# mims-harvard/GNNDelete

Hardware: AMD Instinct MI355X
Metric: Del-op train iters/sec (higher is better)
Workload: dtype f32; 1 GPU; synth-collab GCN 2-layer, 5.0% IN edge deletion, full-graph Del step (both_layerwise, mse_mean); num_nodes=235868, in_dim=128, hidden_dim=128, out_dim=64, train_edges_undirected=2122296, df_edges=53057, sdf_edges=1602188, spmm_nnz=1838056, S1=178921, S2=188697, hip_graph=True, matrix_products=fp32 matrix instruction (v_mfma_f32_32x32x2_f32), parallelism=single, ranks_seen=1

## Files before the change

### gnndelete_amd/_lib.py

```python
import ctypes
import os
import re

_HERE = os.path.dirname(os.path.abspath(__file__))
LIB_PATH = os.environ.get('GNNDELETE_HIP_LIB') or os.path.join(_HERE, 'lib', 'libgnndelete_hip.so')
HEADER_PATH = os.path.join(os.path.dirname(_HERE), 'include', 'gnndelete_hip.h')

_i32, _i64, _f32, _f64, _p = ctypes.c_int32, ctypes.c_int64, ctypes.c_float, ctypes.c_double, ctypes.c_void_p

ABI_VERSION = 9

PROTOTYPES = {
    'gd_abi_version': (ctypes.c_int, []),
    'gd_last_error_string': (ctypes.c_char_p, []),
    'gd_build_source_hash': (ctypes.c_char_p, []),
    'gd_matrix_split': (ctypes.c_int, []),
    'gd_set_matrix_split': (ctypes.c_int, [ctypes.c_int]),
    'gd_csr_from_coo_workspace': (_i64, [_i32, _i64]),
    'gd_csr_from_coo': (ctypes.c_int, [_p, _p, _i64, _i32, _p, _p, _p, _p, _p, _i64, _p]),
    'gd_gcn_norm_f32': (ctypes.c_int, [_p, _p, _i32, _p, _p]),
    'gd_spmm_csr_f32': (ctypes.c_int, [_p, _p, _p, _p, _i64, _p, _i64, _p, _f32, _i32, _i32, _p]),
    'gd_spmm_csr_balanced_f32': (ctypes.c_int, [_p, _i32, _p, _i32, _p, _p, _p, _i64, _p, _i64, _p, _f32, _p, _p, _i32,
                                                _i32, _i32, _p, _p]),
    'gd_spmm_csr_onepass_f32': (ctypes.c_int, [_p, _i32, _p, _p, _p, _i64, _p, _i64, _p, _f32, _p, _i32, _i32, _i32, _p, _p]),
# ... 46 lines not shown
    'gd_batch_loss_terms_workspace': (_i64, [_i32, _i64]),
    'gd_batch_loss_terms': (ctypes.c_int, [_p, _i64, _p, _i64, _i32, _p, _i32, _i32, _f32, _f32, _p, _p, _p, _p, _p, _i64, _p]),
    'gd_rowpair_mse_workspace': (_i64, [_i32]),
    'gd_rowpair_mse_f32': (ctypes.c_int, [_p, _i64, _p, _i64, _i32, _p, _p, _i32, _p, _p, _p, _p, _i64, _i32,
                                          _p, _p, _p]),
    'gd_rowtarget_mse_workspace': (_i64, [_i32]),
    'gd_rowtarget_mse_f32': (ctypes.c_int, [_p, _i64, _p, _i32, _p, _p, _p, _p, _i32, _p, _i64, _p, _p, _p]),
    'gd_rowtarget_mse_pair_covers': (ctypes.c_int32, [_i32, _i32]),
    'gd_rowtarget_mse_pair_f32': (ctypes.c_int, [_p, _i64, _p, _i32, _p, _p, _p, _p, _i32, _p, _i64, _p, _p, _i64, _p, _i32, _p, _p, _p, _p, _i32, _p, _i64, _p, _p]),
    'gd_gemm_f32_workspace': (_i64, [_i32, _i32, _i32]),
    'gd_gemm_f32': (ctypes.c_int, [_p, _i64, _p, _i32, _p, _i32, _i32, _p, _p, _i64, _p, _p]),
    'gd_edge_dot_f32': (ctypes.c_int, [_p, _i64, _i32, _p, _p, _p, _i64, _p, _i64, _p, _p]),
    'gd_edge_dot_bwd_f32': (ctypes.c_int, [_p, _i64, _i32, _p, _p, _p, _i64, _p, _p, _i64, _p, _i64, _p]),
    'gd_rows_gemm_wgrad_adam_f32': (ctypes.c_int, [_p, _i64, _p, _p, _i64, _p, _p, _p, _i32, _i32, _i32, _p, _i32, _p,
                                                   _p, _p, _p, _p, _f64, _f64, _f64, _f64, _p]),
    'gd_rows_gemm_wgrad_blocks': (_i32, [_i32]),
    'gd_rows_gemm_wgrad_loss_f32': (ctypes.c_int, [_p, _i64, _p, _p, _i64, _p, _p, _p, _p, _p, _p, _i32, _i32, _i32, _p, _i32,
                                                   _p, _p, _p, _p, _p, _p, _f64, _f64, _f64, _f64, _p]),
    'gd_del_loss_bwd_blocks': (_i32, [_i32]),
    'gd_del_loss_bwd_f32': (ctypes.c_int, [_p, _i64, _p, _i32, _p, _i32, _p, _p, _p, _p, _p, _i64, _p, _i64, _p, _p]),
    'gd_del_loss_bwd_wgrad_f32': (ctypes.c_int, [_p, _i64, _p, _i32, _p, _i32, _p, _p, _p, _p, _p, _i64, _p, _i64, _p, _p, _p]),
    'gd_del_loss_bwd_wgrad_parts': (ctypes.c_int32, [_i32, _i32]),
    'gd_del_loss_bwd_wgrad_parts_f32': (ctypes.c_int, [_p, _i64, _p, _i32, _p, _i32, _p, _p, _p, _p, _p, _i64, _p, _i64, _p, _p, _i32, _p]),
    'gd_del1_loss_wgrad_covers': (ctypes.c_int32, [_i32, _i32]),
    'gd_del1_loss_wgrad_parts': (ctypes.c_int32, [_i32]),
    'gd_del1_chain_loss_wgrad_f32': (ctypes.c_int, [_p, _i64, _p, _i32, _p, _i32, _p, _i64, _p, _p, _p, _p, _p, _p, _i64, _i32, _p, _p, _p, _p, _p, _p, _p, _i32, _p]),
    'gd_del1_loss_wgrad_f32': (ctypes.c_int, [_p, _i64, _p, _i32, _p, _i32, _p, _i64, _p, _p, _p, _p, _p, _p, _i64, _p, _p, _i32, _p]),
    'gd_rowtarget_mse_blocks': (_i32, [_i32]),
    'gd_rowfold_loss_blocks': (_i32, [_i32]),
    'gd_rowfold_loss_f32': (ctypes.c_int, [_i32, _p, _i64, _p, _i32, _i32, _p, _p, _p, _p, _i32, _p, _i64, _p, _p]),
    'gd_rowfold_kld_scale_f32': (ctypes.c_int, [_p, _i32, _f32, _f32, _f32, _f32, _p, _p, _i32, _i32, _p, _i64, _p, _p]),
    'gd_loss_finalize_f32': (ctypes.c_int, [_p, _i32, _p, _i32, _p, _p, _i32, _p, _p, _p]),
    'gd_pairs_sigmoid_mse_workspace': (_i64, [_i32, _i32]),
    'gd_pairs_sigmoid_mse_f32': (ctypes.c_int, [_p, _i64, _p, _i32, _i32, _p, _i64, _f32, _p, _p, _p, _p]),
    'gd_edgeprob_dec_workspace': (_i64, [_i64, _i32]),
    'gd_edgeprob_dec_f32': (ctypes.c_int, [_p, _i64, _i64, _i32, _p, _i64, _p, _i64, _i64, _f32, _p, _p, _p, _p, _p, _p, _p]),
    'gd_edge_incidence_workspace': (_i64, [_i64, _i64]),
    'gd_edge_incidence': (ctypes.c_int, [_p, _p, _i64, _i64, _p, _p, _p, _p, _i64, _p]),
    'gd_rows_add_f32': (ctypes.c_int, [_p, _i64, _i64, _p, _i32, _p, _i64, _f32, _i32, _p]),
    'gd_edgeprob_record_f32': (ctypes.c_int, [_p, _p, _f32, _f32, _p, _i32, _p, _p]),
    'gd_edge_bce_workspace': (_i64, [_i64, _i32]),
    'gd_edge_bce_f32': (ctypes.c_int, [_p, _i64, _i64, _i32, _p, _i64, _i64, _p, _i64, _i64, _f32, _p, _p, _p, _p, _p, _p, _p]),
    'gd_col_sum_workspace': (_i64, [_i64, _i32]),
    'gd_col_sum_f32': (ctypes.c_int, [_p, _i64, _i64, _i32, _p, _p, _p, _p, _p, _p]),
    'gd_row_nll_workspace': (_i64, [_i64, _i32]),
    'gd_row_nll_f32': (ctypes.c_int, [_p, _i64, _i64, _i32, _i32, _p, _i64, _p, _f32, _p, _i64, _p, _p, _p]),
# ... 74 lines not shown
```

### gnndelete_amd/csrc/del_fused.hip

```cpp
#include <stdlib.h>

#include "common.h"

namespace gd {

using f32x16 = __attribute__((ext_vector_type(16))) float;

struct DelLoss {
  const int32_t* slot;
  const float* tm;
  const float* coef;
  const float* cnt_signed;
  float* partials;
};

template <int NT, bool WG>
__global__ __launch_bounds__(256, (NT == 2 && WG) ? 1 : 2) void del_loss_bwd_kernel(const float* __restrict__ p, int64_t ld_p,
                                                              const int32_t* __restrict__ idx, int32_t n_sel,
                                                              const float* __restrict__ w, DelLoss loss,
                                                              float* __restrict__ dz, int64_t ld_dz,
                                                              float* __restrict__ dp, int64_t ld_dp,
                                                              float* __restrict__ wg_partials) {
  constexpr int D = 32 * NT;
  constexpr int PB = D + 4;
// ... 199 lines not shown
    float* const red = wl;
#pragma unroll
    for (int mt = 0; mt < NT; ++mt)
#pragma unroll
      for (int nt = 0; nt < NT; ++nt)
#pragma unroll
        for (int r = 0; r < 16; ++r)
          red[wave * D * D + (32 * mt + (r & 3) + 8 * (r >> 2) + 4 * kh) * D + 32 * nt + lo] = gacc[mt * NT + nt][r];
    __syncthreads();
    float* const out = wg_partials + (int64_t)blockIdx.x * D * D;
    for (int e = tid; e < D * D; e += 256) out[e] = (red[e] + red[D * D + e]) + (red[2 * D * D + e] + red[3 * D * D + e]);
  }
  ls0 = wave_sum(ls0);
  ls1 = wave_sum(ls1);
  if (lane == 0) { lred[0][wave] = ls0; lred[1][wave] = ls1; }
  __syncthreads();
  if (tid == 0) {
    loss.partials[2 * blockIdx.x + 0] = (lred[0][0] + lred[0][1]) + (lred[0][2] + lred[0][3]);
    loss.partials[2 * blockIdx.x + 1] = (lred[1][0] + lred[1][1]) + (lred[1][2] + lred[1][3]);
  }
}

typedef float f32x4w __attribute__((ext_vector_type(4)));
template <bool HAS_DZ>
__global__ __launch_bounds__(256) __attribute__((amdgpu_waves_per_eu(1, 1))) void del_loss_bwd_ws_kernel(
    const float* __restrict__ p, int64_t ld_p, const int32_t* __restrict__ idx, int32_t n_sel, const float* __restrict__ w,
    DelLoss loss, float* __restrict__ dz, int64_t ld_dz, float* __restrict__ dp, int64_t ld_dp, float* __restrict__ wg_partials,
    int32_t n_part) {
  constexpr int D = 64, PT = 80;
  extern __shared__ __attribute__((aligned(16))) float wl[];
  __shared__ float lred[2][4];
  const int tid = threadIdx.x, lane = tid & 63;
  const int wave = __builtin_amdgcn_readfirstlane(tid >> 6);
  const int r = lane & 15, kq = lane >> 4;
  float* const tp = wl + wave * (2 * 16 * PT);
  float* const tz = tp + 16 * PT;
  const int n_units = (n_sel + 15) >> 4;
  const int n_waves = gridDim.x * 4, wid = blockIdx.x * 4 + wave;
  const int u_lo = (int)((int64_t)n_units * wid / n_waves), u_hi = (int)((int64_t)n_units * (wid + 1) / n_waves);

  auto slot_of = [&](int u) -> int { return min(min(u, n_units - 1) * 16 + r, n_sel - 1); };
  int32_t row_n = idx[slot_of(u_lo)], ls_n = loss.slot[slot_of(u_lo)];
  int32_t row_nn = idx[slot_of(u_lo + 1)], ls_nn = loss.slot[slot_of(u_lo + 1)];
  __builtin_amdgcn_sched_barrier(0);
  float wr1[4][16], wr2[4][16];
#pragma unroll
  for (int t = 0; t < 4; ++t)
#pragma unroll
    for (int s_ = 0; s_ < 16; ++s_) wr1[t][s_] = w[(kq * 16 + s_) * D + 16 * t + r];
#pragma unroll
  for (int t2 = 0; t2 < 4; ++t2)
#pragma unroll
    for (int t = 0; t < 4; ++t) {
      const float4 f = *reinterpret_cast<const float4*>(w + (16 * t2 + r) * D + 16 * t + 4 * kq);
      wr2[t2][4 * t + 0] = f.x; wr2[t2][4 * t + 1] = f.y; wr2[t2][4 * t + 2] = f.z; wr2[t2][4 * t + 3] = f.w;
    }
  f32x4w gacc[16];
#pragma unroll
  for (int i = 0; i < 16; ++i) gacc[i] = f32x4w{0.f, 0.f, 0.f, 0.f};
  float ls0 = 0.f, ls1 = 0.f;

  float4 x[4], tv[4];
  float cf_raw, cn_raw;
  int32_t ls_cur;
  auto fetch_targets = [&](int32_t u) {
    const int uc = max(u, 0);
    const float* trow = loss.tm + (int64_t)uc * D + 4 * kq;
#pragma unroll
    for (int t = 0; t < 4; ++t) tv[t] = *reinterpret_cast<const float4*>(trow + 16 * t);
    cf_raw = loss.coef[uc];
    cn_raw = loss.cnt_signed[uc];
    ls_cur = u;
  };
  auto fetch_rows = [&](int32_t row) {
    const float4* src = reinterpret_cast<const float4*>(p + (int64_t)row * ld_p + kq * 16);
#pragma unroll
    for (int i = 0; i < 4; ++i) x[i] = src[i];
  };
  float a_op[4][4], b_op[4][4];
// ... 14 lines not shown
    fetch_rows(row_n);
    fetch_targets(ls_n);
    for (int u = u_lo; u < u_hi; ++u) {
      const int32_t row = row_n;
      const int s_a = min(u, n_units - 1) * 16 + r;
      const float livef = s_a < n_sel ? 1.f : 0.f;
      row_n = row_nn;
      ls_n = ls_nn;
      row_nn = idx[slot_of(u + 2)];
      ls_nn = loss.slot[slot_of(u + 2)];
      f32x4w acc[4];
#pragma unroll
      for (int i = 0; i < 4; ++i) {
        const float xv[4] = {x[i].x, x[i].y, x[i].z, x[i].w};
#pragma unroll
        for (int c = 0; c < 4; ++c)
#pragma unroll
          for (int t = 0; t < 4; ++t) {
            if (i == 0 && c == 0) acc[t] = __builtin_amdgcn_mfma_f32_16x16x4f32(wr1[t][0], xv[0], f32x4w{0.f, 0.f, 0.f, 0.f}, 0, 0, 0);
            else acc[t] = __builtin_amdgcn_mfma_f32_16x16x4f32(wr1[t][4 * i + c], xv[c], acc[t], 0, 0, 0);
          }
      }
      __builtin_amdgcn_sched_barrier(0);
      p3();
      const float cf = ls_cur >= 0 ? cf_raw : 0.f, cn = ls_cur >= 0 ? cn_raw : 0.f;
      float sq = 0.f;
      f32x4w g[4];
#pragma unroll
      for (int t = 0; t < 4; ++t) {
        const float4 d4 = make_float4(acc[t][0] - tv[t].x, acc[t][1] - tv[t].y, acc[t][2] - tv[t].z, acc[t][3] - tv[t].w);
        sq = fmaf(d4.x, d4.x, sq); sq = fmaf(d4.y, d4.y, sq); sq = fmaf(d4.z, d4.z, sq); sq = fmaf(d4.w, d4.w, sq);
        g[t] = f32x4w{cf * d4.x, cf * d4.y, cf * d4.z, cf * d4.w};
        if (HAS_DZ) *reinterpret_cast<float4*>(dz + (int64_t)min(s_a, n_sel - 1) * ld_dz + 16 * t + 4 * kq) = make_float4(g[t][0], g[t][1], g[t][2], g[t][3]);
        *reinterpret_cast<float4*>(tz + r * PT + 16 * t + 4 * kq) = make_float4(livef * g[t][0], livef * g[t][1], livef * g[t][2], livef * g[t][3]);
      }
      sq *= livef;
      if (cn >= 0.f) ls0 = fmaf(cn, sq, ls0); else ls1 = fmaf(-cn, sq, ls1);
#pragma unroll
      for (int i = 0; i < 4; ++i) *reinterpret_cast<float4*>(tp + r * PT + kq * 16 + 4 * i) = x[i];
      __builtin_amdgcn_sched_barrier(0);
      fetch_targets(ls_n);
      fetch_rows(row_n);
      __builtin_amdgcn_fence(__ATOMIC_ACQ_REL, "wavefront");
      __builtin_amdgcn_wave_barrier();
#pragma unroll
      for (int sp = 0; sp < 4; ++sp)
#pragma unroll
        for (int t = 0; t < 4; ++t) {
          a_op[sp][t] = tp[(4 * sp + kq) * PT + 16 * t + r];
          b_op[sp][t] = tz[(4 * sp + kq) * PT + 16 * t + r];
        }
      __builtin_amdgcn_sched_barrier(0);
      f32x4w dacc[4];
#pragma unroll
      for (int t = 0; t < 4; ++t)
#pragma unroll
        for (int c = 0; c < 4; ++c)
#pragma unroll
          for (int t2 = 0; t2 < 4; ++t2) {
            if (t == 0 && c == 0) dacc[t2] = __builtin_amdgcn_mfma_f32_16x16x4f32(wr2[t2][0], g[0][0], f32x4w{0.f, 0.f, 0.f, 0.f}, 0, 0, 0);
            else dacc[t2] = __builtin_amdgcn_mfma_f32_16x16x4f32(wr2[t2][4 * t + c], g[t][c], dacc[t2], 0, 0, 0);
          }
      __builtin_amdgcn_sched_barrier(0);
      {
        float* orow = dp + (int64_t)row * ld_dp + 4 * kq;
#pragma unroll
        for (int t2 = 0; t2 < 4; ++t2) *reinterpret_cast<float4*>(orow + 16 * t2) = make_float4(dacc[t2][0], dacc[t2][1], dacc[t2][2], dacc[t2][3]);
      }
      __builtin_amdgcn_fence(__ATOMIC_ACQ_REL, "wavefront");
      __builtin_amdgcn_wave_barrier();
      __builtin_amdgcn_sched_barrier(0);
    }
    p3();
  }
  __syncthreads();
  float* const red = wl;
#pragma unroll
  for (int ta = 0; ta < 4; ++ta)
#pragma unroll
    for (int tb = 0; tb < 4; ++tb)
#pragma unroll
      for (int v = 0; v < 4; ++v) red[wave * D * D + (16 * ta + 4 * kq + v) * D + 16 * tb + r] = gacc[ta * 4 + tb][v];
  __syncthreads();
  for (int slot = blockIdx.x; slot < n_part; slot += gridDim.x) {
    float* const out = wg_partials + (int64_t)slot * D * D;
    const bool mine = slot == (int)blockIdx.x;
    for (int e = tid; e < D * D; e += 256) out[e] = mine ? (red[e] + red[D * D + e]) + (red[2 * D * D + e] + red[3 * D * D + e]) : 0.f;
  }
  ls0 = wave_sum(ls0);
  ls1 = wave_sum(ls1);
  if (lane == 0) { lred[0][wave] = ls0; lred[1][wave] = ls1; }
  __syncthreads();
  if (tid == 0) {
    for (int slot = blockIdx.x; slot < n_part; slot += gridDim.x) {
      const bool mine = slot == (int)blockIdx.x;
      loss.partials[2 * slot + 0] = mine ? (lred[0][0] + lred[0][1]) + (lred[0][2] + lred[0][3]) : 0.f;
// ... 423 lines not shown
  hipStream_t s = (hipStream_t)stream;
  const DelLoss loss{loss_slot, tm, coef, cnt_signed, loss_partials};
  if (!with_wgrad) {
    const dim3 grid(del_fused_grid(n_sel));
    const size_t lds = ((size_t)d * d + (size_t)d * (d + 4)) * sizeof(float);
    switch (d / 32) {
      case 1: hipLaunchKernelGGL((del_loss_bwd_kernel<1, false>), grid, dim3(256), lds, s, p, ld_p, idx, n_sel, w, loss, dz, ld_dz, dp, ld_dp, nullptr); break;
      default: hipLaunchKernelGGL((del_loss_bwd_kernel<2, false>), grid, dim3(256), lds, s, p, ld_p, idx, n_sel, w, loss, dz, ld_dz, dp, ld_dp, nullptr); break;
    }
    return launched("del_loss_bwd");
  }
  static const bool ws_on = [] { const char* e = getenv("GD_DEL2_WS"); return !(e && atoi(e) == 0); }();
  if (ws_on && d == 64 && n_sel >= 65536) {
    const int n_all = gd_rows_gemm_wgrad_blocks(n_sel);
    const int n_part = n_part_req > 0 ? n_part_req : n_all;
    GD_REQUIRE(n_part <= n_all && n_part >= (ws_cu_count() < n_all ? ws_cu_count() : n_all), GD_E_DIM,
               "%s: n_part=%d outside [gd_del_loss_bwd_wgrad_parts, gd_rows_gemm_wgrad_blocks = %d]", name, n_part, n_all);
    const int grid_ws = ws_cu_count() < n_part ? ws_cu_count() : n_part;
    constexpr int kLdsWs = 4 * 64 * 64 * 4;
    if (dz) {
      static const hipError_t a1 = hipFuncSetAttribute(reinterpret_cast<const void*>(&del_loss_bwd_ws_kernel<true>), hipFuncAttributeMaxDynamicSharedMemorySize, kLdsWs);
      if (a1 != hipSuccess) return fail(-(int)a1, "gd_del_loss_bwd_wgrad_f32: %s", hipGetErrorString(a1));
      hipLaunchKernelGGL((del_loss_bwd_ws_kernel<true>), dim3(grid_ws), dim3(256), kLdsWs, s, p, ld_p, idx, n_sel, w, loss, dz, ld_dz, dp, ld_dp,
                         wgrad_partials, n_part);
    } else {
      static const hipError_t a0 = hipFuncSetAttribute(reinterpret_cast<const void*>(&del_loss_bwd_ws_kernel<false>), hipFuncAttributeMaxDynamicSharedMemorySize, kLdsWs);
      if (a0 != hipSuccess) return fail(-(int)a0, "gd_del_loss_bwd_wgrad_f32: %s", hipGetErrorString(a0));
      hipLaunchKernelGGL((del_loss_bwd_ws_kernel<false>), dim3(grid_ws), dim3(256), kLdsWs, s, p, ld_p, idx, n_sel, w, loss, dz, ld_dz, dp, ld_dp,
                         wgrad_partials, n_part);
    }
    return launched("del_loss_bwd_ws");
  }
  GD_REQUIRE(n_part_req == 0 || n_part_req == gd_rows_gemm_wgrad_blocks(n_sel), GD_E_DIM,
             "%s: n_part=%d but this size leaves gd_rows_gemm_wgrad_blocks(n_sel) = %d partials", name, n_part_req, gd_rows_gemm_wgrad_blocks(n_sel));
  const dim3 grid(gd_rows_gemm_wgrad_blocks(n_sel));
#define GD_DF_CASE(NT_)                                                                                                        \
  do {                                                                                                                         \
    constexpr int kD = 32 * NT_;                                                                                               \
    constexpr int kLds = (kD * kD + kD * (kD + 4) + 4 * 32 * (kD + 4)) * 4;                                                    \
    static_assert(kLds >= 4 * kD * kD * 4, "block sum needs 4 D^2 floats");                                                    \
    static const hipError_t attr = hipFuncSetAttribute(reinterpret_cast<const void*>(&del_loss_bwd_kernel<NT_, true>),         \
                                                       hipFuncAttributeMaxDynamicSharedMemorySize, kLds);                      \
    if (attr != hipSuccess) return fail(-(int)attr, "gd_del_loss_bwd_wgrad_f32: %s", hipGetErrorString(attr));                 \
    hipLaunchKernelGGL((del_loss_bwd_kernel<NT_, true>), grid, dim3(256), kLds, s, p, ld_p, idx, n_sel, w, loss, dz, ld_dz,    \
                       dp, ld_dp, wgrad_partials);                                                                             \
  } while (0)
  if (d == 32) GD_DF_CASE(1); else GD_DF_CASE(2);
#undef GD_DF_CASE
  return launched("del_loss_bwd_wgrad");
}

extern "C" int gd_del_loss_bwd_f32(const float* p, int64_t ld_p, const int32_t* idx, int32_t n_sel, const float* w,
// ... 7 lines not shown
extern "C" int gd_del_loss_bwd_wgrad_f32(const float* p, int64_t ld_p, const int32_t* idx, int32_t n_sel, const float* w,
                                         int32_t d, const int32_t* loss_slot, const float* tm, const float* coef,
                                         const float* cnt_signed, float* dz, int64_t ld_dz, float* dp, int64_t ld_dp,
                                         float* loss_partials, float* wgrad_partials, void* stream) {
  return del_loss_bwd_impl(p, ld_p, idx, n_sel, w, d, loss_slot, tm, coef, cnt_signed, dz, ld_dz, dp, ld_dp, loss_partials,
                           wgrad_partials, true, stream);
}

extern "C" int32_t gd_del_loss_bwd_wgrad_parts(int32_t n_sel, int32_t d) {
  if (n_sel <= 0) return 0;
  const int nb = gd_rows_gemm_wgrad_blocks(n_sel);
  static const bool ws_on = [] { const char* e = getenv("GD_DEL2_WS"); return !(e && atoi(e) == 0); }();
  if (ws_on && d == 64 && n_sel >= 65536) return gd::ws_cu_count() < nb ? gd::ws_cu_count() : nb;
  return nb;
}

extern "C" int gd_del_loss_bwd_wgrad_parts_f32(const float* p, int64_t ld_p, const int32_t* idx, int32_t n_sel, const float* w, int32_t d,
                                               const int32_t* loss_slot, const float* tm, const float* coef, const float* cnt_signed,
                                               float* dz, int64_t ld_dz, float* dp, int64_t ld_dp, float* loss_partials,
                                               float* wgrad_partials, int32_t n_part, void* stream) {
  GD_REQUIRE(n_part > 0 || n_sel == 0, GD_E_DIM, "gd_del_loss_bwd_wgrad_parts_f32: n_part=%d", n_part);
  return del_loss_bwd_impl(p, ld_p, idx, n_sel, w, d, loss_slot, tm, coef, cnt_signed, dz, ld_dz, dp, ld_dp, loss_partials,
                           wgrad_partials, true, stream, n_part);
}

extern "C" int32_t gd_del1_loss_wgrad_covers(int32_t n_sel, int32_t d) {
  static const bool on = [] { const char* e = getenv("GD_DEL1_FUSED"); return !(e && atoi(e) == 0); }();
  return on && d == 128 && n_sel >= 65536 ? 1 : 0;
}

extern "C" int32_t gd_del1_loss_wgrad_parts(int32_t n_sel) {
  if (n_sel <= 0) return 0;
  const int nb = gd_rows_gemm_wgrad_blocks(n_sel);
  return gd::ws_cu_count() < nb ? gd::ws_cu_count() : nb;
}

extern "C" int gd_del1_loss_wgrad_f32(const float* p, int64_t ld_p, const int32_t* idx, int32_t n_sel, const float* w, int32_t d,
                                      float* z, int64_t ld_z, uint32_t* sign_out, const int32_t* loss_slot, const float* tm,
                                      const float* coef, const float* cnt_signed, const float* g_add, int64_t ld_gadd,
                                      float* loss_partials, float* wgrad_partials, int32_t n_part, void* stream) {
  using namespace gd;
  const char* name = "gd_del1_loss_wgrad_f32";
  if (n_sel == 0) return GD_OK;
  GD_REQUIRE(p && idx && w && z && sign_out && loss_slot && tm && coef && cnt_signed && loss_partials && wgrad_partials, GD_E_NULL,
             "%s: null pointer", name);
  GD_REQUIRE(d == 128, GD_E_DIM, "%s: d=%d must be 128 (other widths: gd_rows_gemm_signs_f32 + gd_rows_gemm_wgrad_loss_f32)", name, d);
// ... 64 lines not shown
```

### gnndelete_amd/engine.py

```python
import os
import warnings
from typing import NamedTuple

import torch

from . import _lib, ops
from ._lib import check, ptr, stream_ptr
from .capture import capture_iterations
from .graph import graph_for
from .nn import GATConv, GCNConv, GINConv, RGCNConv, SAGEConv

LOSS_TYPES = ('both_all', 'both_layerwise', 'only2_layerwise', 'only2_all', 'only1')


class StepFacts(NamedTuple):
    mode: str
    loss_type: str
    family: str
    h: int
    o: int
    s1: int
    s2: int
    folded1: bool
    n_rows1: int
# ... 68 lines not shown
     closed, w2_mfma, gin_ok, del1_covers, pair_covers) = facts
    mse = family == 'mse'
    mixed_ok = folded1 and folded2 and not k.no_split_loss and not k.no_split
    out2 = not inside2 and mixed_ok and mse and s2 > 0 and o in (32, 64) and n_rows2 > 0 and not k.no_fused_l2
    split2 = (inside2 or out2) and not k.no_split
    fuse_l2 = mse and split2 and folded1 and o in (32, 64) and n_rows2 > 0 and not k.no_fused_l2
    split1 = (not cache_layer1 or k.cache_split) and inside1 and not k.no_split
    loss1_ok = (mse and folded1 and folded2 and loss_type in ('both_layerwise', 'both_all', 'only1') and s1 > 0
                and h in (32, 64, 128) and n_rows1 > 0 and not k.no_fused_loss1)
    out1 = loss1_ok and not inside1 and mixed_ok
    fuse_loss1 = loss1_ok and (inside1 or out1)
    tail = (folded1 and folded2 and s1 > 0 and s2 > 0 and loss_type in ('both_layerwise', 'both_all') and h % 2 == 0 and o % 2 == 0
            and not k.no_step_tail
            and ((fuse_loss1 and fuse_l2) or (h in (32, 64, 128) and o in (32, 64, 128) and not k.tail_fused_only)))
    fuse_wg2 = tail and fuse_l2 and not k.no_fused_wgrad2
    fuse_del1 = tail and fuse_loss1 and split1 and loss_type in ('both_layerwise', 'only1') and del1_covers
    chain1 = (fuse_del1 and loss_type == 'both_layerwise' and h == 128 and o == 64 and k.del1_chain
              and (mode in ('gcn', 'gin') or (mode == 'gat' and w2_mfma and not k.no_gat_rank1_epilogue)))
    out_pair = out1 and out2 and fuse_loss1 and fuse_l2 and loss_type != 'only2_all' and pair_covers and not k.no_loss_pair
    rows_only = (rows_only_asked and (mode in ('gcn', 'gat', 'sage') or gin_ok) and split2 and s2 > 0
                 and not out1 and not out2 and closed)
    return StepForms(split1, split2, out1, out2, fuse_loss1, fuse_l2, tail, fuse_wg2, fuse_del1, chain1, out_pair, rows_only,
                     rows_only_asked and mode == 'rgcn', not k.no_gat_dots)


def _loss_coefficients(loss_type, alpha):
    if loss_type in ('both_all', 'both_layerwise', 'only2_layerwise'):
        return alpha, 1.0 - alpha
    return alpha, 1.0


LOSS_FAMILIES = {'mse_mean': ('mse', 'mean'), 'mse_sum': ('mse', 'sum'), 'kld_mean': ('kld', 'mean'), 'kld_sum': ('kld', 'sum'),
                 'cosine_mean': ('cosine', 'mean'), 'cosine_sum': ('cosine', 'sum')}
_ROWFOLD_FAMILY = {'cosine': 0, 'kld': 1}


def fold_row_terms(family, z_ori, rows, tgt, kind, d_valid=None):
    assert family in ('kld', 'cosine'), family
    d = z_ori.shape[1]
    dv = d if d_valid is None else int(d_valid)
    device = z_ori.device
    uniq, inv, c = torch.unique(rows, return_inverse=True, return_counts=True)
    kind_u = torch.zeros(uniq.numel(), dtype=torch.int32, device=device)
    kind_u[inv] = kind.to(torch.int32)
    if uniq.numel() == 0:
        return uniq, torch.zeros(0, d, dtype=torch.float64, device=device), c, kind_u, [0.0, 0.0]
# ... 386 lines not shown
        self.g2 = torch.zeros_like(self.wd2)
        self.sums = torch.zeros(4, **f32)
        self.ws1 = torch.empty(max(1, lib.gd_rows_gemm_wgrad_workspace(self.s1, self.h, self.h)), **f32)
        self.ws2 = torch.empty(max(1, lib.gd_rows_gemm_wgrad_workspace(self.s2, self.o, self.o)), **f32)
        self.iter_ctr = torch.zeros(1, dtype=torch.int32, device=dev)
        self.adam1, self.adam2 = _Adam(self.wd1, lr, iter_ctr=self.iter_ctr), _Adam(self.wd2, lr, iter_ctr=self.iter_ctr)
        self.hist = torch.zeros(history, 4, **f32)
        self.hist_pos = torch.zeros(1, dtype=torch.int32, device=dev)
        self.steps_done = 0
        self._graph = self._graph_k = None
        self._use_graph = use_graph
        self._const_refs = {}
        if self._fuse_loss1:
            self._slot1, self._cnt_signed1 = _loss_slots(self.t1, self.idx1, self.s1, dev)
            self._lp1_blocks = lib.gd_del1_loss_wgrad_parts(self.s1) if self._fuse_del1 else lib.gd_rows_gemm_wgrad_blocks(self.s1)
            self._lp1 = torch.zeros(2 * max(1, lib.gd_rows_gemm_wgrad_blocks(self.s1) + self.t1.outside_blocks()), **f32)
        self._tail_acc = [0, 0]
        self._arrive = torch.zeros(2, dtype=torch.int32, device=dev)
        self._gat_bufs = self._dt2_keep = None
        if self._chain1 and self._mode == 'gat':
            self._gat_bufs = {'dh': torch.zeros(n, self.o, **f32), 'da_src': torch.zeros(n, **f32), 'da_dst': torch.zeros(n, **f32)}
        elif self._chain1:
            self._dt2_keep = torch.zeros(n, self.o, **f32)
        self._gat_r1 = None
        if self._mode == 'gat':
            w2_ = conv2.lin_src.weight.detach()
            self._gat_r1 = ((conv2.att_src.detach().reshape(1, -1) @ w2_).reshape(-1).float().contiguous(),
                            (conv2.att_dst.detach().reshape(1, -1) @ w2_).reshape(-1).float().contiguous())
        if self._mode == 'rgcn':
            from .graph import TypedNodeCSR
            self.typed = TypedNodeCSR(edge_index, edge_type.to(dev), n, conv2.num_relations)
            self.typed_s1 = None
            if self._rgcn_rows_only and self.s1 > 0:
                in1 = torch.zeros(n, dtype=torch.bool, device=dev)
                in1[self.idx1.long()] = True
                self.typed_s1 = self.typed.restrict_bwd(in1)
            self._hbuf = torch.zeros(n, self.h, **f32)
            self._dxbuf = torch.zeros(n, self.h, **f32)
            for c_, din, dout, tr in ((conv1, self.x.shape[1], self.h, 0), (conv2, self.h, self.o, 0), (conv2, self.o, self.h, 1)):
                if int(lib.gd_rgcn_tile_kl(din, dout, c_.num_blocks or 1, tr)) > 0 and not knobs.rgcn_node_major:
                    tg_ = self.typed_s1 if (tr and self.typed_s1 is not None) else self.typed
                    if ops.rgcn_wave_form(din, dout, c_.num_blocks or 1, n, din) and self.typed.num_relations < 65536:
                        tg_.wave_plan(bool(tr))
                    else:
                        tg_.tile_plan(bool(tr))
                    ops.rgcn_packed_weight(c_.weight.detach(), c_.num_blocks or 1, din, dout, tr)
# ... 298 lines not shown
                      else (self.t1.partials, self.t1.n_partial_blocks()))
            p2, n2 = ((self._lp2, self._lp2_blocks + (self.t2.outside_blocks() if self._out2 else 0)) if self._fuse_l2
                      else (self.t2.partials, self.t2.n_partial_blocks()))
            if self._tail:
                a1, a2 = self.adam1, self.adam2
                lib_ = _lib.lib()
                nw1 = self._lp1_blocks if self._fuse_del1 else lib_.gd_rows_gemm_wgrad_blocks(self.s1)
                check(lib_.gd_step_tail_parts_f32(
                    ptr(self.ws1), nw1, self.h, self._tail_acc[0], ptr(self.g1), ptr(a1.param), ptr(a1.m), ptr(a1.v),
                    ptr(self.ws2), self._lp2_blocks if self._fuse_wg2 else lib_.gd_rows_gemm_wgrad_blocks(self.s2), self.o,
                    self._tail_acc[1], ptr(self.g2), ptr(a2.param),
                    ptr(a2.m), ptr(a2.v), a1.lr, a1.betas[0], a1.betas[1], a1.eps, ptr(p1), n1, ptr(p2), n2, ptr(self.hist),
                    self.hist.shape[0], ptr(self.hist_pos), ptr(self.iter_ctr), ptr(self._arrive), stream_ptr(self.x.device)),
                    'gd_step_tail_parts_f32')
            else:
                check(_lib.lib().gd_loss_finalize_f32(
                    ptr(p1) if fused_fin else None, n1 if fused_fin else 0,
                    ptr(p2) if fused_fin else None, n2 if fused_fin else 0,
                    None if fused_fin else ptr(self.sums), ptr(self.hist), self.hist.shape[0], ptr(self.hist_pos),
                    ptr(self.iter_ctr), stream_ptr(self.x.device)), 'gd_loss_finalize_f32')
            if self._user_wd2 is not None:
                self._user_wd2.data.copy_(self.wd2.data[:self._o_true, :self._o_true])

    def _del1_fused(self, g_add):
        self.adam1.applied += 1
        self._tail_acc[0] = 0
        if self._chain1:
            c2 = self.model.conv2
            if self._mode == 'gat':
                w_next, dt = c2.lin_src.weight.detach(), self._gat_bufs['dh']
                rank1 = (ptr(self._gat_bufs['da_src']), ptr(self._gat_r1[0]), ptr(self._gat_bufs['da_dst']), ptr(self._gat_r1[1]))
            else:
                w_next, dt = (c2.lin if self._mode == 'gcn' else c2.nn).weight.detach(), self._dt2_keep
                rank1 = (None, None, None, None)
            check(_lib.lib().gd_del1_chain_loss_wgrad_f32(
                ptr(self.pre1), self.pre1.stride(0), ptr(self.idx1), self.s1, ptr(self.wd1), self.h, ptr(self.z1), self.z1.stride(0),
                ptr(self.z1_pos), ptr(self._slot1), ptr(self.t1.tm), ptr(self.t1.coef), ptr(self._cnt_signed1), ptr(dt),
                dt.stride(0), self.o, ptr(w_next), *rank1, ptr(self._lp1), ptr(self.ws1), self._lp1_blocks,
                stream_ptr(self.x.device)), 'gd_del1_chain_loss_wgrad_f32')
            return
        check(_lib.lib().gd_del1_loss_wgrad_f32(
            ptr(self.pre1), self.pre1.stride(0), ptr(self.idx1), self.s1, ptr(self.wd1), self.h, ptr(self.z1), self.z1.stride(0),
            ptr(self.z1_pos), ptr(self._slot1), ptr(self.t1.tm), ptr(self.t1.coef), ptr(self._cnt_signed1), ptr(g_add),
            g_add.stride(0) if g_add is not None else 0, ptr(self._lp1), ptr(self.ws1), self._lp1_blocks, stream_ptr(self.x.device)),
            'gd_del1_loss_wgrad_f32')

    def _del2_fused(self):
        if self._fuse_wg2:
            check(_lib.lib().gd_del_loss_bwd_wgrad_parts_f32(
                ptr(self.p2), self.p2.stride(0), ptr(self.idx2), self.s2, ptr(self.wd2), self.o, ptr(self._slot2),
                ptr(self.t2.tm), ptr(self.t2.coef), ptr(self._cnt_signed2), None, self.o,
                ptr(self.dz2), self.dz2.stride(0), ptr(self._lp2), ptr(self.ws2), self._lp2_blocks, stream_ptr(self.x.device)),
                'gd_del_loss_bwd_wgrad_parts_f32')
            return
        check(_lib.lib().gd_del_loss_bwd_f32(
            ptr(self.p2), self.p2.stride(0), ptr(self.idx2), self.s2, ptr(self.wd2), self.o, ptr(self._slot2),
            ptr(self.t2.tm), ptr(self.t2.coef), ptr(self._cnt_signed2), ptr(self.dz2c), self.dz2c.stride(0),
            ptr(self.dz2), self.dz2.stride(0), ptr(self._lp2), stream_ptr(self.x.device)), 'gd_del_loss_bwd_f32')

    def _layer2_backward(self, to_w1=True, g2_accumulate=False):
        if self._fuse_wg2:
            self.adam2.applied += 1
            self._tail_acc[1] = int(g2_accumulate)
        elif self._fuse_l2:
            self._wgrad(self.p2, self.dz2c, None, self.s2, self.g2, g2_accumulate, self.ws2, a_idx=self.idx2,
                        adam=self.adam2)
        elif self._split2:
            self._wgrad(self.p2, self.dz2, self.idx2, self.s2, self.g2, g2_accumulate, self.ws2, a_idx=self.idx2,
                        adam=self.adam2 if self._tail else None)
        else:
# ... 23 lines not shown
        if n_steps >= unroll:
            self.prepare_unrolled(unroll)
            while n_steps >= unroll:
                self._graph_k[1].replay()
                self.steps_done += unroll
                n_steps -= unroll
        for _ in range(n_steps):
            self.step()

    def prepare_unrolled(self, unroll):
        if not self._use_graph or unroll <= 1:
            return
        if self._graph is None:
            self._capture()
        if self._graph_k is None or self._graph_k[0] != unroll:
            self._graph_k = (unroll, capture_iterations(self._iteration, self._mutable_state, unroll, warm_up=False))

    def _mutable_state(self):
        state = [self.wd1.data, self.wd2.data, self.g1, self.g2, self.adam1.m, self.adam1.v, self.iter_ctr,
                 self.adam2.m, self.adam2.v, self.hist, self.hist_pos, self.dz1, self.dz2, self.dh]
        if self._chain1:
            state += [self.z1_pos] + ([self._dt2_keep] if self._dt2_keep is not None else
                                      [self._gat_bufs[k] for k in ('dh', 'da_src', 'da_dst')])
        state.append(self._arrive)
        if self._user_wd2 is not None:
            state.append(self._user_wd2.data)
        return state

    def _capture(self):
        self._graph = capture_iterations(self._iteration, self._mutable_state)

    def loss_history(self):
        k = min(self.steps_done, self.hist.shape[0])
        s = self.hist[:k].double().cpu()
        nan = float('nan')
        fam = self.family
        r1 = logged_loss(fam, s[:, 0], self.t1.k_const[0], self.t1.n_r) if self.t1.count_r else s[:, 0] * nan
        l1 = logged_loss(fam, s[:, 1], self.t1.k_const[1], self.t1.n_l) if self.t1.count_l else s[:, 1] * nan
        r2 = logged_loss(fam, s[:, 2], self.t2.k_const[0], self.t2.n_r) if self.t2.count_r else s[:, 2] * nan
        l2 = logged_loss(fam, s[:, 3], self.t2.k_const[1], self.t2.n_l) if self.t2.count_l else s[:, 3] * nan
        a, lt = self.alpha, self.loss_type
        if lt in ('both_all', 'both_layerwise'):
            loss_r, loss_l = r1 + r2, l1 + l2
            loss = a * loss_r + (1 - a) * loss_l
        elif lt == 'only2_layerwise':
            loss_r, loss_l = r1 + r2, l1 + l2
# ... 9 lines not shown
```

### include/gnndelete_hip.h

```cpp
#ifndef GNNDELETE_HIP_H
#define GNNDELETE_HIP_H

#include <stdint.h>

#ifdef __cplusplus
extern "C" {
#endif

#define GD_ABI_VERSION 9

enum {
  GD_OK = 0,
  GD_E_NULL = 1,
  GD_E_DIM = 2,
  GD_E_ALIGN = 3,
  GD_E_WORKSPACE = 4
};

int gd_abi_version(void);
const char* gd_last_error_string(void);
const char* gd_build_source_hash(void);

#define GD_MATRIX_SPLIT_DEFAULT 0
int gd_matrix_split(void);
// ... 174 lines not shown
int gd_rows_gemm_wgrad_loss_f32(const float* a, int64_t ld_a, const int32_t* a_idx,
                                const float* z, int64_t ld_z, const int32_t* z_idx,
                                const int32_t* loss_slot, const float* tm, const float* coef,
                                const float* cnt_signed, const float* g_add,
                                int32_t n_sel, int32_t d_a, int32_t d_b, float* dw, int32_t accumulate,
                                float* partials, float* loss_partials,
                                float* param, float* exp_avg, float* exp_avg_sq, const int32_t* iter,
                                double lr, double beta1, double beta2, double eps, void* stream);

int32_t gd_del_loss_bwd_blocks(int32_t n_sel);
int gd_del_loss_bwd_f32(const float* p, int64_t ld_p, const int32_t* idx, int32_t n_sel, const float* w, int32_t d,
                        const int32_t* loss_slot, const float* tm, const float* coef, const float* cnt_signed,
                        float* dz, int64_t ld_dz, float* dp, int64_t ld_dp, float* loss_partials, void* stream);

int gd_del_loss_bwd_wgrad_f32(const float* p, int64_t ld_p, const int32_t* idx, int32_t n_sel, const float* w, int32_t d,
                              const int32_t* loss_slot, const float* tm, const float* coef, const float* cnt_signed,
                              float* dz, int64_t ld_dz, float* dp, int64_t ld_dp, float* loss_partials,
                              float* wgrad_partials, void* stream);
int32_t gd_del_loss_bwd_wgrad_parts(int32_t n_sel, int32_t d);
int gd_del_loss_bwd_wgrad_parts_f32(const float* p, int64_t ld_p, const int32_t* idx, int32_t n_sel, const float* w, int32_t d,
                                    const int32_t* loss_slot, const float* tm, const float* coef, const float* cnt_signed,
                                    float* dz, int64_t ld_dz, float* dp, int64_t ld_dp, float* loss_partials,
                                    float* wgrad_partials, int32_t n_part, void* stream);

int32_t gd_del1_loss_wgrad_covers(int32_t n_sel, int32_t d);
int32_t gd_del1_loss_wgrad_parts(int32_t n_sel);
int gd_del1_loss_wgrad_f32(const float* p, int64_t ld_p, const int32_t* idx, int32_t n_sel, const float* w, int32_t d, float* z,
                           int64_t ld_z, uint32_t* sign_out, const int32_t* loss_slot, const float* tm, const float* coef,
                           const float* cnt_signed, const float* g_add, int64_t ld_gadd, float* loss_partials,
                           float* wgrad_partials, int32_t n_part, void* stream);
int gd_del1_chain_loss_wgrad_f32(const float* p, int64_t ld_p, const int32_t* idx, int32_t n_sel, const float* w, int32_t d, float* z,
                                 int64_t ld_z, uint32_t* sign_io, const int32_t* loss_slot, const float* tm, const float* coef,
                                 const float* cnt_signed, const float* dt, int64_t ld_dt, int32_t d_next, const float* w_next,
                                 const float* row_a, const float* col_a, const float* row_b, const float* col_b,
                                 float* loss_partials, float* wgrad_partials, int32_t n_part, void* stream);


int64_t gd_rowpair_mse_workspace(int32_t n_seg);
int gd_rowpair_mse_f32(const float* z, int64_t ld_z, const float* o, int64_t ld_o, int32_t d,
                       const int32_t* seg_ptr, const int32_t* seg_row, int32_t n_seg,
                       const int32_t* term_o, const float* term_w, const int32_t* term_kind,
                       float* dz, int64_t ld_dz, int32_t dz_compact,
                       float* sums, float* partials, void* stream);

int64_t gd_rowtarget_mse_workspace(int32_t n_rows);
int gd_rowtarget_mse_f32(const float* z, int64_t ld_z, const float* tm, int32_t d,
// ... 124 lines not shown
```

Before: 1898 iters/s.

## Fold layer-2 deletion weight into next-layer weight to skip per-row backward GEMM

Adds a FOLD variant of the layer-2 deletion loss/backward kernel. Instead of multiplying each selected row's gradient by the deletion weight (a per-row MFMA GEMM written to dp), it writes the raw scaled gradient and has some blocks compute W_fold = W_del^T · W_conv2 once (a 64x128 product). The layer-1 chain kernel then consumes W_fold in place of the conv2 weight, removing one per-row GEMM over S2 rows. This reorders the algebra, which can change rounding slightly, and adds a small serial tail at the end of the kernel for the fold product.

```diff
diff --git a/gnndelete_amd/_lib.py b/gnndelete_amd/_lib.py
--- a/gnndelete_amd/_lib.py
+++ b/gnndelete_amd/_lib.py
@@ -92,6 +92,8 @@
     'gd_del_loss_bwd_wgrad_f32': (ctypes.c_int, [_p, _i64, _p, _i32, _p, _i32, _p, _p, _p, _p, _p, _i64, _p, _i64, _p, _p, _p]),
     'gd_del_loss_bwd_wgrad_parts': (ctypes.c_int32, [_i32, _i32]),
     'gd_del_loss_bwd_wgrad_parts_f32': (ctypes.c_int, [_p, _i64, _p, _i32, _p, _i32, _p, _p, _p, _p, _p, _i64, _p, _i64, _p, _p, _i32, _p]),
+    'gd_del_loss_fold_wgrad_covers': (ctypes.c_int32, [_i32, _i32, _i32]),
+    'gd_del_loss_fold_wgrad_parts_f32': (ctypes.c_int, [_p, _i64, _p, _i32, _p, _i32, _p, _p, _p, _p, _p, _i64, _p, _i32, _p, _p, _p, _i32, _p]),
     'gd_del1_loss_wgrad_covers': (ctypes.c_int32, [_i32, _i32]),
     'gd_del1_loss_wgrad_parts': (ctypes.c_int32, [_i32]),
     'gd_del1_chain_loss_wgrad_f32': (ctypes.c_int, [_p, _i64, _p, _i32, _p, _i32, _p, _i64, _p, _p, _p, _p, _p, _p, _i64, _i32, _p, _p, _p, _p, _p, _p, _p, _i32, _p]),
diff --git a/gnndelete_amd/csrc/del_fused.hip b/gnndelete_amd/csrc/del_fused.hip
--- a/gnndelete_amd/csrc/del_fused.hip
+++ b/gnndelete_amd/csrc/del_fused.hip
@@ -245,11 +245,13 @@
 }
 
 typedef float f32x4w __attribute__((ext_vector_type(4)));
-template <bool HAS_DZ>
+struct DelFold { const float* w_next; float* w_fold; };
+constexpr int kFoldH = 128;
+template <bool HAS_DZ, bool FOLD = false>
 __global__ __launch_bounds__(256) __attribute__((amdgpu_waves_per_eu(1, 1))) void del_loss_bwd_ws_kernel(
     const float* __restrict__ p, int64_t ld_p, const int32_t* __restrict__ idx, int32_t n_sel, const float* __restrict__ w,
     DelLoss loss, float* __restrict__ dz, int64_t ld_dz, float* __restrict__ dp, int64_t ld_dp, float* __restrict__ wg_partials,
-    int32_t n_part) {
+    int32_t n_part, DelFold fold) {
   constexpr int D = 64, PT = 80;
   extern __shared__ __attribute__((aligned(16))) float wl[];
   __shared__ float lred[2][4];
@@ -266,18 +268,20 @@
   int32_t row_n = idx[slot_of(u_lo)], ls_n = loss.slot[slot_of(u_lo)];
   int32_t row_nn = idx[slot_of(u_lo + 1)], ls_nn = loss.slot[slot_of(u_lo + 1)];
   __builtin_amdgcn_sched_barrier(0);
-  float wr1[4][16], wr2[4][16];
+  float wr1[4][16], wr2[FOLD ? 1 : 4][16];
 #pragma unroll
   for (int t = 0; t < 4; ++t)
 #pragma unroll
     for (int s_ = 0; s_ < 16; ++s_) wr1[t][s_] = w[(kq * 16 + s_) * D + 16 * t + r];
-#pragma unroll
-  for (int t2 = 0; t2 < 4; ++t2)
-#pragma unroll
-    for (int t = 0; t < 4; ++t) {
-      const float4 f = *reinterpret_cast<const float4*>(w + (16 * t2 + r) * D + 16 * t + 4 * kq);
-      wr2[t2][4 * t + 0] = f.x; wr2[t2][4 * t + 1] = f.y; wr2[t2][4 * t + 2] = f.z; wr2[t2][4 * t + 3] = f.w;
-    }
+  if (!FOLD) {
+#pragma unroll
+    for (int t2 = 0; t2 < 4; ++t2)
+#pragma unroll
+      for (int t = 0; t < 4; ++t) {
+        const float4 f = *reinterpret_cast<const float4*>(w + (16 * t2 + r) * D + 16 * t + 4 * kq);
+        wr2[t2][4 * t + 0] = f.x; wr2[t2][4 * t + 1] = f.y; wr2[t2][4 * t + 2] = f.z; wr2[t2][4 * t + 3] = f.w;
+      }
+  }
   f32x4w gacc[16];
 #pragma unroll
   for (int i = 0; i < 16; ++i) gacc[i] = f32x4w{0.f, 0.f, 0.f, 0.f};
@@ -338,6 +342,12 @@
           }
       }
       __builtin_amdgcn_sched_barrier(0);
+      if (FOLD) {
+#pragma unroll
+        for (int i = 0; i < 4; ++i) *reinterpret_cast<float4*>(tp + r * PT + kq * 16 + 4 * i) = x[i];
+        __builtin_amdgcn_sched_barrier(0);
+        fetch_rows(row_n);
+      }
       p3();
       const float cf = ls_cur >= 0 ? cf_raw : 0.f, cn = ls_cur >= 0 ? cn_raw : 0.f;
       float sq = 0.f;
@@ -348,15 +358,18 @@
         sq = fmaf(d4.x, d4.x, sq); sq = fmaf(d4.y, d4.y, sq); sq = fmaf(d4.z, d4.z, sq); sq = fmaf(d4.w, d4.w, sq);
         g[t] = f32x4w{cf * d4.x, cf * d4.y, cf * d4.z, cf * d4.w};
         if (HAS_DZ) *reinterpret_cast<float4*>(dz + (int64_t)min(s_a, n_sel - 1) * ld_dz + 16 * t + 4 * kq) = make_float4(g[t][0], g[t][1], g[t][2], g[t][3]);
+        if (FOLD) *reinterpret_cast<float4*>(dp + (int64_t)row * ld_dp + 16 * t + 4 * kq) = make_float4(g[t][0], g[t][1], g[t][2], g[t][3]);
         *reinterpret_cast<float4*>(tz + r * PT + 16 * t + 4 * kq) = make_float4(livef * g[t][0], livef * g[t][1], livef * g[t][2], livef * g[t][3]);
       }
       sq *= livef;
       if (cn >= 0.f) ls0 = fmaf(cn, sq, ls0); else ls1 = fmaf(-cn, sq, ls1);
-#pragma unroll
-      for (int i = 0; i < 4; ++i) *reinterpret_cast<float4*>(tp + r * PT + kq * 16 + 4 * i) = x[i];
+      if (!FOLD) {
+#pragma unroll
+        for (int i = 0; i < 4; ++i) *reinterpret_cast<float4*>(tp + r * PT + kq * 16 + 4 * i) = x[i];
+      }
       __builtin_amdgcn_sched_barrier(0);
       fetch_targets(ls_n);
-      fetch_rows(row_n);
+      if (!FOLD) fetch_rows(row_n);
       __builtin_amdgcn_fence(__ATOMIC_ACQ_REL, "wavefront");
       __builtin_amdgcn_wave_barrier();
 #pragma unroll
@@ -367,18 +380,18 @@
           b_op[sp][t] = tz[(4 * sp + kq) * PT + 16 * t + r];
         }
       __builtin_amdgcn_sched_barrier(0);
-      f32x4w dacc[4];
-#pragma unroll
-      for (int t = 0; t < 4; ++t)
-#pragma unroll
-        for (int c = 0; c < 4; ++c)
-#pragma unroll
-          for (int t2 = 0; t2 < 4; ++t2) {
-            if (t == 0 && c == 0) dacc[t2] = __builtin_amdgcn_mfma_f32_16x16x4f32(wr2[t2][0], g[0][0], f32x4w{0.f, 0.f, 0.f, 0.f}, 0, 0, 0);
-            else dacc[t2] = __builtin_amdgcn_mfma_f32_16x16x4f32(wr2[t2][4 * t + c], g[t][c], dacc[t2], 0, 0, 0);
-          }
-      __builtin_amdgcn_sched_barrier(0);
-      {
+      if (!FOLD) {
+        f32x4w dacc[4];
+#pragma unroll
+        for (int t = 0; t < 4; ++t)
+#pragma unroll
+          for (int c = 0; c < 4; ++c)
+#pragma unroll
+            for (int t2 = 0; t2 < 4; ++t2) {
+              if (t == 0 && c == 0) dacc[t2] = __builtin_amdgcn_mfma_f32_16x16x4f32(wr2[t2][0], g[0][0], f32x4w{0.f, 0.f, 0.f, 0.f}, 0, 0, 0);
+              else dacc[t2] = __builtin_amdgcn_mfma_f32_16x16x4f32(wr2[t2][4 * t + c], g[t][c], dacc[t2], 0, 0, 0);
+            }
+        __builtin_amdgcn_sched_barrier(0);
         float* orow = dp + (int64_t)row * ld_dp + 4 * kq;
 #pragma unroll
         for (int t2 = 0; t2 < 4; ++t2) *reinterpret_cast<float4*>(orow + 16 * t2) = make_float4(dacc[t2][0], dacc[t2][1], dacc[t2][2], dacc[t2][3]);
@@ -388,6 +401,18 @@
       __builtin_amdgcn_sched_barrier(0);
     }
     p3();
+  }
+  if (FOLD) {
+    const int nb = min((int)gridDim.x, D * kFoldH / 256);
+    if ((int)blockIdx.x < nb) {
+      for (int e = blockIdx.x * 256 + tid; e < D * kFoldH; e += nb * 256) {
+        const int i = e / kFoldH, n = e % kFoldH;
+        float acc = 0.f;
+#pragma unroll 16
+        for (int c = 0; c < D; ++c) acc = fmaf(w[c * D + i], fold.w_next[c * kFoldH + n], acc);
+        fold.w_fold[e] = acc;
+      }
+    }
   }
   __syncthreads();
   float* const red = wl;
@@ -857,12 +882,12 @@
       static const hipError_t a1 = hipFuncSetAttribute(reinterpret_cast<const void*>(&del_loss_bwd_ws_kernel<true>), hipFuncAttributeMaxDynamicSharedMemorySize, kLdsWs);
       if (a1 != hipSuccess) return fail(-(int)a1, "gd_del_loss_bwd_wgrad_f32: %s", hipGetErrorString(a1));
       hipLaunchKernelGGL((del_loss_bwd_ws_kernel<true>), dim3(grid_ws), dim3(256), kLdsWs, s, p, ld_p, idx, n_sel, w, loss, dz, ld_dz, dp, ld_dp,
-                         wgrad_partials, n_part);
+                         wgrad_partials, n_part, DelFold{nullptr, nullptr});
     } else {
       static const hipError_t a0 = hipFuncSetAttribute(reinterpret_cast<const void*>(&del_loss_bwd_ws_kernel<false>), hipFuncAttributeMaxDynamicSharedMemorySize, kLdsWs);
       if (a0 != hipSuccess) return fail(-(int)a0, "gd_del_loss_bwd_wgrad_f32: %s", hipGetErrorString(a0));
       hipLaunchKernelGGL((del_loss_bwd_ws_kernel<false>), dim3(grid_ws), dim3(256), kLdsWs, s, p, ld_p, idx, n_sel, w, loss, dz, ld_dz, dp, ld_dp,
-                         wgrad_partials, n_part);
+                         wgrad_partials, n_part, DelFold{nullptr, nullptr});
     }
     return launched("del_loss_bwd_ws");
   }
@@ -916,6 +941,38 @@
   GD_REQUIRE(n_part > 0 || n_sel == 0, GD_E_DIM, "gd_del_loss_bwd_wgrad_parts_f32: n_part=%d", n_part);
   return del_loss_bwd_impl(p, ld_p, idx, n_sel, w, d, loss_slot, tm, coef, cnt_signed, dz, ld_dz, dp, ld_dp, loss_partials,
                            wgrad_partials, true, stream, n_part);
+}
+
+extern "C" int32_t gd_del_loss_fold_wgrad_covers(int32_t n_sel, int32_t d, int32_t h) {
+  static const bool ws_on = [] { const char* e = getenv("GD_DEL2_WS"); return !(e && atoi(e) == 0); }();
+  return ws_on && d == 64 && h == gd::kFoldH && n_sel >= 65536 ? 1 : 0;
+}
+
+extern "C" int gd_del_loss_fold_wgrad_parts_f32(const float* p, int64_t ld_p, const int32_t* idx, int32_t n_sel, const float* w, int32_t d,
+                                                const int32_t* loss_slot, const float* tm, const float* coef, const float* cnt_signed,
+                                                float* g, int64_t ld_g, const float* w_next, int32_t h, float* w_fold,
+                                                float* loss_partials, float* wgrad_partials, int32_t n_part, void* stream) {
+  using namespace gd;
+  const char* name = "gd_del_loss_fold_wgrad_parts_f32";
+  GD_REQUIRE(gd_del_loss_fold_wgrad_covers(n_sel, d, h), GD_E_DIM,
+             "%s: n_sel=%d, d=%d, h=%d is not covered (gd_del_loss_fold_wgrad_covers: d = 64, h = 128, >= 65,536 rows)", name, n_sel, d, h);
+  GD_REQUIRE(p && idx && w && loss_slot && tm && coef && cnt_signed && g && w_next && w_fold && loss_partials && wgrad_partials, GD_E_NULL,
+             "%s: null pointer", name);
+  GD_REQUIRE(ld_p >= d && ld_g >= d && ld_p % 4 == 0 && ld_g % 4 == 0, GD_E_DIM, "%s: bad row strides", name);
+  GD_REQUIRE(aligned16(p) && aligned16(tm) && aligned16(g) && aligned16(w) && aligned16(w_fold) && aligned16(wgrad_partials), GD_E_ALIGN,
+             "%s: unaligned", name);
+  GD_REQUIRE(p != g && w_fold != w && w_fold != w_next, GD_E_DIM, "%s: buffers must not alias", name);
+  const int n_all = gd_rows_gemm_wgrad_blocks(n_sel);
+  GD_REQUIRE(n_part <= n_all && n_part >= (ws_cu_count() < n_all ? ws_cu_count() : n_all), GD_E_DIM,
+             "%s: n_part=%d outside [gd_del_loss_bwd_wgrad_parts, gd_rows_gemm_wgrad_blocks = %d]", name, n_part, n_all);
+  const int grid_ws = ws_cu_count() < n_part ? ws_cu_count() : n_part;
+  constexpr int kLdsWs = 4 * 64 * 64 * 4;
+  static const hipError_t at = hipFuncSetAttribute(reinterpret_cast<const void*>(&del_loss_bwd_ws_kernel<false, true>), hipFuncAttributeMaxDynamicSharedMemorySize, kLdsWs);
+  if (at != hipSuccess) return fail(-(int)at, "%s: %s", name, hipGetErrorString(at));
+  const DelLoss loss{loss_slot, tm, coef, cnt_signed, loss_partials};
+  hipLaunchKernelGGL((del_loss_bwd_ws_kernel<false, true>), dim3(grid_ws), dim3(256), kLdsWs, (hipStream_t)stream, p, ld_p, idx, n_sel, w, loss,
+                     static_cast<float*>(nullptr), (int64_t)0, g, ld_g, wgrad_partials, n_part, DelFold{w_next, w_fold});
+  return launched("del_loss_fold_ws");
 }
 
 extern "C" int32_t gd_del1_loss_wgrad_covers(int32_t n_sel, int32_t d) {
diff --git a/gnndelete_amd/engine.py b/gnndelete_amd/engine.py
--- a/gnndelete_amd/engine.py
+++ b/gnndelete_amd/engine.py
@@ -114,6 +114,15 @@
                  and not out1 and not out2 and closed)
     return StepForms(split1, split2, out1, out2, fuse_loss1, fuse_l2, tail, fuse_wg2, fuse_del1, chain1, out_pair, rows_only,
                      rows_only_asked and mode == 'rgcn', not k.no_gat_dots)
+
+
+def read_del2_fold(env=None):
+    env = os.environ if env is None else env
+    return env.get('GD_DEL2_FOLD') != '0'
+
+
+def plan_del2_fold(facts, forms, covers, enabled=True):
+    return bool(enabled and covers and forms.chain1 and facts.mode in ('gcn', 'gin') and forms.fuse_wg2 and not forms.out2)
 
 
 def _loss_coefficients(loss_type, alpha):
@@ -546,6 +555,8 @@
             self._gat_bufs = {'dh': torch.zeros(n, self.o, **f32), 'da_src': torch.zeros(n, **f32), 'da_dst': torch.zeros(n, **f32)}
         elif self._chain1:
             self._dt2_keep = torch.zeros(n, self.o, **f32)
+        self._fold2 = plan_del2_fold(self.facts, self.forms, lib.gd_del_loss_fold_wgrad_covers(self.s2, self.o, self.h), read_del2_fold())
+        self._w2fold = torch.zeros(self.o, self.h, **f32) if self._fold2 else None
         self._gat_r1 = None
         if self._mode == 'gat':
             w2_ = conv2.lin_src.weight.detach()
@@ -890,6 +901,10 @@
             if self._user_wd2 is not None:
                 self._user_wd2.data.copy_(self.wd2.data[:self._o_true, :self._o_true])
 
+    def _conv2_weight(self):
+        c2 = self.model.conv2
+        return (c2.lin if self._mode == 'gcn' else c2.nn).weight.detach()
+
     def _del1_fused(self, g_add):
         self.adam1.applied += 1
         self._tail_acc[0] = 0
@@ -899,7 +914,9 @@
                 w_next, dt = c2.lin_src.weight.detach(), self._gat_bufs['dh']
                 rank1 = (ptr(self._gat_bufs['da_src']), ptr(self._gat_r1[0]), ptr(self._gat_bufs['da_dst']), ptr(self._gat_r1[1]))
             else:
-                w_next, dt = (c2.lin if self._mode == 'gcn' else c2.nn).weight.detach(), self._dt2_keep
+                w_next, dt = self._conv2_weight(), self._dt2_keep
+                if self._fold2:
+                    w_next = self._w2fold
                 rank1 = (None, None, None, None)
             check(_lib.lib().gd_del1_chain_loss_wgrad_f32(
                 ptr(self.pre1), self.pre1.stride(0), ptr(self.idx1), self.s1, ptr(self.wd1), self.h, ptr(self.z1), self.z1.stride(0),
@@ -914,6 +931,14 @@
             'gd_del1_loss_wgrad_f32')
 
     def _del2_fused(self):
+        if self._fold2:
+            w2 = self._conv2_weight()
+            check(_lib.lib().gd_del_loss_fold_wgrad_parts_f32(
+                ptr(self.p2), self.p2.stride(0), ptr(self.idx2), self.s2, ptr(self.wd2), self.o, ptr(self._slot2),
+                ptr(self.t2.tm), ptr(self.t2.coef), ptr(self._cnt_signed2), ptr(self.dz2), self.dz2.stride(0), ptr(w2), self.h,
+                ptr(self._w2fold), ptr(self._lp2), ptr(self.ws2), self._lp2_blocks, stream_ptr(self.x.device)),
+                'gd_del_loss_fold_wgrad_parts_f32')
+            return
         if self._fuse_wg2:
             check(_lib.lib().gd_del_loss_bwd_wgrad_parts_f32(
                 ptr(self.p2), self.p2.stride(0), ptr(self.idx2), self.s2, ptr(self.wd2), self.o, ptr(self._slot2),
@@ -983,6 +1008,8 @@
         if self._chain1:
             state += [self.z1_pos] + ([self._dt2_keep] if self._dt2_keep is not None else
                                       [self._gat_bufs[k] for k in ('dh', 'da_src', 'da_dst')])
+        if self._fold2:
+            state.append(self._w2fold)
         state.append(self._arrive)
         if self._user_wd2 is not None:
             state.append(self._user_wd2.data)
diff --git a/include/gnndelete_hip.h b/include/gnndelete_hip.h
--- a/include/gnndelete_hip.h
+++ b/include/gnndelete_hip.h
@@ -220,6 +220,11 @@
                                     const int32_t* loss_slot, const float* tm, const float* coef, const float* cnt_signed,
                                     float* dz, int64_t ld_dz, float* dp, int64_t ld_dp, float* loss_partials,
                                     float* wgrad_partials, int32_t n_part, void* stream);
+int32_t gd_del_loss_fold_wgrad_covers(int32_t n_sel, int32_t d, int32_t h);
+int gd_del_loss_fold_wgrad_parts_f32(const float* p, int64_t ld_p, const int32_t* idx, int32_t n_sel, const float* w, int32_t d,
+                                     const int32_t* loss_slot, const float* tm, const float* coef, const float* cnt_signed,
+                                     float* g, int64_t ld_g, const float* w_next, int32_t h, float* w_fold,
+                                     float* loss_partials, float* wgrad_partials, int32_t n_part, void* stream);
 
 int32_t gd_del1_loss_wgrad_covers(int32_t n_sel, int32_t d);
 int32_t gd_del1_loss_wgrad_parts(int32_t n_sel);
```

Result: faster. 1921 iters/s, median of 6 (+1.2%).
